# eladb3/SViT

Hardware: AMD Instinct MI355X
Metric: clips/sec (fwd+bwd) SViT 16x224^2 bf16 (higher is better)
Workload: dtype bf16; 1 GPU; SViT 16x224^2, 8 clips/GPU, 4 object tokens/frame, fwd+CE+bwd+clip+AdamW; global_batch=8, parallelism=dp1, ranks_seen=1, forced_dp=False, launch=hip-graph replay, input=fp32 clips, resident in the replayed step's input buffers, hip_library=svit_amd/lib/libsvit_hip.so

## Files before the change

include/svit_hip.h:

```cpp
#ifndef SVIT_HIP_H
#define SVIT_HIP_H
#include <stdint.h>
#ifdef __cplusplus
extern "C" {
#endif

#define SVIT_HEAD_DIM 96

int svit_version(void);
const char* svit_arch(void);

enum {
  SVIT_EPI_BF16 = 0,
  SVIT_EPI_GELU = 1,
  SVIT_EPI_RESID = 2,
  SVIT_EPI_F32 = 3,
  SVIT_EPI_DGELU = 4,
  SVIT_EPI_RELQ = 5
};
typedef struct {
  const void* A; int32_t lda;
  const void* W; int32_t ldw;
  const float* bias;
  void* out; int32_t ldo;
  void* out2; int32_t ldo2;
  const void* aux; int32_t ldaux;
  const float* row_scale; int32_t rows_per_sample;
  int32_t M, N, K;
  int32_t epilogue; int32_t accumulate;
  int32_t remap_L, remap_N, remap_off;
  const int32_t* relq_map;
  void* relq_out; int32_t relq_ld;
  int32_t relq_extra, relq_rows;
  float relq_scale;
} svit_gemm_args;
int svit_gemm_nt(const svit_gemm_args* args, void* stream);
int svit_gemm_tn(const void* A, int lda, const void* B, int ldb, float* dW, int lddw,
                 int M, int N, int K, int splits, float* dbias ,
                 void* stream);
#define SVIT_TN_GROUP_MAX 16
typedef struct {
  const void* A; const void* B; float* dW; float* dbias;
  int32_t lda, ldb, lddw, M, N, K;
} svit_tn_problem;
int svit_gemm_tn_grouped(const svit_tn_problem* probs, int count, void* stream);
int svit_gemm_tn_grouped_ex(const svit_tn_problem* probs, int count, int ordered, void* stream);
int svit_gemm_tn_grouped_slab(const svit_tn_problem* probs, int count, float* workspace,
                              int64_t workspace_floats, void* stream);
int64_t svit_gemm_tn_grouped_workspace(const svit_tn_problem* probs, int count);
int svit_gemm_tn_grouped_slab_lead(const svit_tn_problem* probs, int count, int launch_count, float* workspace,
                                   int64_t workspace_floats, void* stream);
// ... 297 lines not shown
int svit_ce_loss_soft(const float* logits, const float* target, const int64_t* labels, const void* mix, float on,
                      float off, int B, int C, float* loss, float* dlogits, void* stream);
int svit_step_draws(uint64_t* state, const float* keep, int n_blocks, int per_block, float* scales,
                    int n_drop, float p_drop, float* drop, void* stream);

int svit_ensemble_update(const float* preds, const int64_t* labels, const int64_t* clip_ids,
                         int N, int C, int num_clips, int num_videos, int mode, int repeat,
                         float* video_preds, int64_t* video_labels, int64_t* clip_count,
                         int* err, void* stream);
int svit_topk_correct(const float* video_preds, const int64_t* video_labels, int V, int C,
                      const int* ks, int nk, int* counts, int* err, void* stream);
#define SVIT_METER_MAX_SCALARS 16
int svit_meter_push(float* ring, int W, int K, int64_t* state, const float* const* scalars, int n_scalars,
                    const float* logits, const int64_t* labels, int N, int C, int k0, int k1, void* stream);
int svit_debug_set(int key, int val);
int svit_debug_gemm_nt_plan(int M, int N, int K, int epilogue, int32_t* out, int n_out);
int svit_debug_set_tn(int step_us_x100, int atomic_tbs_x100);
int svit_debug_set_tn_tile(int mode);
int svit_debug_gemm_tn_plan(const svit_tn_problem* probs, int count, int form, int arg, int64_t* out, int n_out);
int svit_debug_set_pool(int key, int val);
int svit_debug_pool_bwd_path(void);
int svit_debug_pool_plan(int kind, int B, int heads, int T, int H, int W, int n_obj, int sq, int sk, int sv, int save_mask,
                         int sel, int relq_lpad, int32_t* out, int n_out);
int svit_attn_debug_set(int key, int val);
int svit_debug_reset(void);
#ifdef __cplusplus
}
#endif
#endif
```

svit_amd/build.py:

```python
import concurrent.futures
import os
import re
import subprocess
import sys

HERE = os.path.dirname(os.path.abspath(__file__))
CSRC = os.path.join(HERE, "csrc")
OUT_DIR = os.path.join(HERE, "lib")
LIB = os.path.join(OUT_DIR, "libsvit_hip.so")
SOURCES = ["gemm_nt.hip", "gemm_tn.hip", "norm.hip", "misc.hip", "pool.hip", "attn_fwd.hip", "attn_bwd.hip",
           "loss.hip", "meter.hip", "input.hip", "head.hip", "randaug.hip", "feed.hip", "head_eval.hip", "solver.hip",
           "monitor.hip", "actmon.hip"]
HEADERS = ["common.h", "attn_common.h", "gemm_epilogue.h", os.path.join("..", "..", "include", "svit_hip.h")]
HIPCC = os.environ.get("HIPCC", "/opt/rocm/bin/hipcc")
FLAGS = ["--offload-arch=gfx950", "-O3", "-fPIC", "-std=c++17", "-ffast-math",
         "-fno-finite-math-only", "-fno-slp-vectorize", "-Wno-unused-result"]
SOURCE_FLAGS = {"randaug.hip": {"remove": ["-ffast-math"], "add": ["-ffp-contract=off"]}}
TMP_DIR = os.path.join(OUT_DIR, "tmp")


def flags_for(src):
    change = SOURCE_FLAGS.get(src, {})
    return [f for f in FLAGS if f not in change.get("remove", ())] + list(change.get("add", ()))


# ... 115 lines not shown
```

svit_amd/csrc/common.h:

```cpp
#pragma once
#include <hip/hip_runtime.h>
#include <stdint.h>

typedef uint16_t bf16_t;
typedef __bf16 bf16x8_t __attribute__((ext_vector_type(8)));
typedef __bf16 bf16x4_t __attribute__((ext_vector_type(4)));
typedef short s16x4_t __attribute__((ext_vector_type(4)));
typedef short s16x8_t __attribute__((ext_vector_type(8)));
typedef float f32x16_t __attribute__((ext_vector_type(16)));
typedef float f32x4_t __attribute__((ext_vector_type(4)));

#define SVIT_OK 0
#define SVIT_ERR_SHAPE (-2)
#define SVIT_ERR_ALIGN (-3)
#define SVIT_ERR_ARG (-4)

struct SvitOnce {
  unsigned long long mask;
};
static inline int svit_max_lds_once(SvitOnce& once, const void* fn, size_t bytes) {
  int dev = 0;
  if (hipGetDevice(&dev) != hipSuccess) dev = 0;
  const unsigned long long bit = 1ull << (dev & 63);
  if (__atomic_load_n(&once.mask, __ATOMIC_ACQUIRE) & bit) return 0;
// ... 4 lines not shown
}

enum SvitKnob {
  SVIT_K_NT_STAGES = 0,
  SVIT_K_NT_CFG,
  SVIT_K_NT_BK,
  SVIT_K_TN_STEP_US_X100,
  SVIT_K_TN_ATOMIC_TBS_X100,
  SVIT_K_TN_TILE,
  SVIT_K_POOL_FWD,
  SVIT_K_POOL_BWD,
  SVIT_K_POOL_FWD_LARGE,
  SVIT_K_ATTN_DKV_FORM,
  SVIT_K_ATTN_FWD_SHORT,
  SVIT_K_POOL_FRAME,
  SVIT_K_COUNT
};
int svit_knob(int k);
int svit_knob_set(int k, int v);
void svit_knob_reset();

#define SVIT_LAUNCH_CHECK()                       \
  do {                                            \
    hipError_t e__ = hipGetLastError();           \
    if (e__ != hipSuccess) return (int)e__;       \
  } while (0)

__device__ __forceinline__ float bf16_to_f32(bf16_t v) {
  return __uint_as_float(((uint32_t)v) << 16);
}
// ... 110 lines not shown
```

svit_amd/csrc/gemm_epilogue.h:

```cpp
#pragma once
#include "common.h"
#ifndef SVIT_EPI_AHEAD
#define SVIT_EPI_AHEAD 1
#endif
#include "../../include/svit_hip.h"

template <bool WAVE_PRIVATE>
__device__ __forceinline__ void nt_epi_sync() {
  if constexpr (WAVE_PRIVATE) asm volatile("s_waitcnt lgkmcnt(0)" ::: "memory");
  else __syncthreads();
}

template <int RB, int NB, int EPI, bool WAVE_PRIVATE = false>
__device__ __forceinline__ void nt_epilogue_wide(const svit_gemm_args& p, f32x16_t (&acc)[RB][NB],
                                                 unsigned char* smem, int m0, int n0, int wm, int wn,
                                                 int lane, int wave) {
  constexpr int WN = 32 * NB, EP_LD = WN + 4, GPR = 4 * NB;
  float* stg = (float*)smem + wave * (16 * EP_LD);
  uint4 aux_ring[3][NB];
  auto fetch_aux = [&](int ih, uint4 (&dst)[NB]) {
    const int i = ih >> 1, half = ih & 1;
#pragma unroll
    for (int it = 0; it < NB; ++it) {
      const int idx = lane + 64 * it, rl = idx / GPR, c8 = idx % GPR;
      const int row = m0 + wm * 32 * RB + i * 32 + half * 16 + rl, col = n0 + wn * WN + c8 * 8;
      dst[it] = make_uint4(0, 0, 0, 0);
      if (row < p.M && col < p.N) dst[it] = *(const uint4*)((const bf16_t*)p.aux + (size_t)row * p.ldaux + col);
    }
  };
  float4 bias_r[NB][2];
#pragma unroll
  for (int it = 0; it < NB; ++it) {
    const int col = n0 + wn * WN + ((lane + 64 * it) % GPR) * 8;
    bias_r[it][0] = bias_r[it][1] = make_float4(0.f, 0.f, 0.f, 0.f);
    if (p.bias && col < p.N) {
      bias_r[it][0] = *(const float4*)(p.bias + col);
      bias_r[it][1] = *(const float4*)(p.bias + col + 4);
    }
  }
  constexpr int AHEAD = SVIT_EPI_AHEAD;
  if (EPI == SVIT_EPI_DGELU) {
    fetch_aux(0, aux_ring[0]);
    if (AHEAD > 1 && 2 * RB > 1) fetch_aux(1, aux_ring[1]);
  }
#pragma unroll
  for (int ih = 0; ih < 2 * RB; ++ih) {
    const int i = ih >> 1, half = ih & 1;
#pragma unroll
    for (int j = 0; j < NB; ++j)
#pragma unroll
      for (int rr = 0; rr < 8; ++rr)
        stg[((rr & 3) + 8 * (rr >> 2) + 4 * (lane >> 5)) * EP_LD + j * 32 + (lane & 31)] =
            acc[i][j][half * 8 + rr];
    if (EPI == SVIT_EPI_DGELU && ih + AHEAD < 2 * RB) fetch_aux(ih + AHEAD, aux_ring[(ih + AHEAD) % 3]);
    nt_epi_sync<WAVE_PRIVATE>();
#pragma unroll
    for (int it = 0; it < NB; ++it) {
      const int idx = lane + 64 * it, rl = idx / GPR, c8 = idx % GPR;
      const int row = m0 + wm * 32 * RB + i * 32 + half * 16 + rl, col = n0 + wn * WN + c8 * 8;
      if (row >= p.M || col >= p.N) continue;
      const float4 v0 = *(const float4*)(stg + rl * EP_LD + c8 * 8), v1 = *(const float4*)(stg + rl * EP_LD + c8 * 8 + 4);
      const float4 b0 = bias_r[it][0], b1 = bias_r[it][1];
      float v[8] = {v0.x + b0.x, v0.y + b0.y, v0.z + b0.z, v0.w + b0.w, v1.x + b1.x, v1.y + b1.y, v1.z + b1.z, v1.w + b1.w};
      uint4 o;
      if constexpr (EPI == SVIT_EPI_BF16) {
        o.x = pack_bf16x2(v[0], v[1]); o.y = pack_bf16x2(v[2], v[3]);
        o.z = pack_bf16x2(v[4], v[5]); o.w = pack_bf16x2(v[6], v[7]);
      } else if constexpr (EPI == SVIT_EPI_GELU) {
        float a[8], d[8];
#pragma unroll
        for (int e = 0; e < 8; ++e) gelu_fwd_grad(v[e], &a[e], &d[e]);
        if (p.out2) {
          uint4 o2;
          o2.x = pack_bf16x2(d[0], d[1]); o2.y = pack_bf16x2(d[2], d[3]);
          o2.z = pack_bf16x2(d[4], d[5]); o2.w = pack_bf16x2(d[6], d[7]);
          *(uint4*)((bf16_t*)p.out2 + (size_t)row * p.ldo2 + col) = o2;
        }
        o.x = pack_bf16x2(a[0], a[1]); o.y = pack_bf16x2(a[2], a[3]);
        o.z = pack_bf16x2(a[4], a[5]); o.w = pack_bf16x2(a[6], a[7]);
      } else {
        const uint4 h = aux_ring[ih % 3][it];
        o.x = pack_bf16x2(v[0] * lo_bf16(h.x), v[1] * hi_bf16(h.x));
        o.y = pack_bf16x2(v[2] * lo_bf16(h.y), v[3] * hi_bf16(h.y));
        o.z = pack_bf16x2(v[4] * lo_bf16(h.z), v[5] * hi_bf16(h.z));
        o.w = pack_bf16x2(v[6] * lo_bf16(h.w), v[7] * hi_bf16(h.w));
      }
      *(uint4*)((bf16_t*)p.out + (size_t)row * p.ldo + col) = o;
    }
    if (ih + 1 < 2 * RB) nt_epi_sync<WAVE_PRIVATE>();
  }
}

template <int RB, int NB>
__device__ __forceinline__ void nt_epilogue_relq(const svit_gemm_args& p, f32x16_t (&acc)[RB][NB],
                                                 unsigned char* smem, int m0, int n0, int wm, int wn,
                                                 int lane, int wave) {
  constexpr int WN = 32 * NB, EP_LD = WN + 4;
  constexpr int MAXV = 16;
  float* stg = (float*)smem + wave * (16 * EP_LD);
  const int extra = p.relq_extra, sh = extra == 64 ? 6 : 5;
  const int nv = 16 * extra / 64;
  const int c_lo = n0 + wn * WN;
// ... 177 lines not shown
```

svit_amd/csrc/misc.hip:

```cpp
#include <cstring>
#include <mutex>
#include <unordered_map>
#include "common.h"
#include "../../include/svit_hip.h"

namespace {

__global__ void cast_kernel(const float* __restrict__ src, bf16_t* __restrict__ dst, int64_t n) {
  const int64_t stride = (int64_t)gridDim.x * blockDim.x * 8;
  for (int64_t i = ((int64_t)blockIdx.x * blockDim.x + threadIdx.x) * 8; i < n; i += stride) {
    if (i + 8 <= n) {
      const float4 a = *(const float4*)(src + i), b = *(const float4*)(src + i + 4);
      uint4 o;
      o.x = pack_bf16x2(a.x, a.y); o.y = pack_bf16x2(a.z, a.w);
      o.z = pack_bf16x2(b.x, b.y); o.w = pack_bf16x2(b.z, b.w);
      *(uint4*)(dst + i) = o;
    } else {
      for (int64_t j = i; j < n; ++j) dst[j] = f32_to_bf16(src[j]);
    }
  }
}

__global__ void transpose_cast_kernel(const float* __restrict__ src_base,
                                      bf16_t* __restrict__ dst_base,
// ... 671 lines not shown
  if (!jobs_dev || n_jobs <= 0 || n_jobs > 65535 || max_rows <= 0) return SVIT_ERR_ARG;
  hipLaunchKernelGGL(table_interp_batched_kernel, dim3(max_rows, n_jobs), dim3(128), 0, (hipStream_t)stream, jobs_dev);
  SVIT_LAUNCH_CHECK();
  return SVIT_OK;
}

extern "C" int svit_table_interp(const float* M, int rows, int J, const float* tables, float* out32, void* out16, void* stream) {
  if (!M || !tables || (!out32 && !out16) || rows <= 0 || J <= 0) return SVIT_ERR_ARG;
  hipLaunchKernelGGL(table_interp_kernel, dim3(rows), dim3(128), 0, (hipStream_t)stream, M, J, tables, out32, (bf16_t*)out16);
  SVIT_LAUNCH_CHECK();
  return SVIT_OK;
}

static const int k_knob_default[SVIT_K_COUNT] = {
     0,  -1,  0,  85,  75,  2,
     2,  1,  1,  0,  1,  2};
static int g_knob[SVIT_K_COUNT] = {0, -1, 0, 85, 75, 2, 2, 1, 1, 0, 1, 2};
int svit_knob(int k) { return __atomic_load_n(&g_knob[k], __ATOMIC_RELAXED); }
int svit_knob_set(int k, int v) {
  if (k < 0 || k >= SVIT_K_COUNT) return SVIT_ERR_ARG;
  __atomic_store_n(&g_knob[k], v, __ATOMIC_RELAXED);
  return SVIT_OK;
}
void svit_knob_reset() {
  for (int k = 0; k < SVIT_K_COUNT; ++k) __atomic_store_n(&g_knob[k], k_knob_default[k], __ATOMIC_RELAXED);
}
extern "C" int svit_debug_set(int key, int val) {
  if (key == 0) return (val == 0 || (val >= 2 && val <= 4)) ? svit_knob_set(SVIT_K_NT_STAGES, val) : SVIT_ERR_ARG;
  if (key == 1) return (val >= -1 && val <= 10) ? svit_knob_set(SVIT_K_NT_CFG, val) : SVIT_ERR_ARG;
  if (key == 2) return (val == 0 || val == 32 || val == 64) ? svit_knob_set(SVIT_K_NT_BK, val) : SVIT_ERR_ARG;
  return SVIT_ERR_ARG;
}
extern "C" int svit_debug_set_tn(int step_us_x100, int atomic_tbs_x100) {
  if (step_us_x100 > 0) svit_knob_set(SVIT_K_TN_STEP_US_X100, step_us_x100);
  if (atomic_tbs_x100 > 0) svit_knob_set(SVIT_K_TN_ATOMIC_TBS_X100, atomic_tbs_x100);
  return SVIT_OK;
}
extern "C" int svit_debug_set_tn_tile(int mode) {
  return (mode >= 0 && mode <= 3) ? svit_knob_set(SVIT_K_TN_TILE, mode) : SVIT_ERR_ARG;
}
extern "C" int svit_debug_set_pool(int key, int val) {
  if (key == 0) return (val >= 0 && val <= 3) ? svit_knob_set(SVIT_K_POOL_FWD, val) : SVIT_ERR_ARG;
  if (key == 1) return (val == 0 || val == 1) ? svit_knob_set(SVIT_K_POOL_BWD, val) : SVIT_ERR_ARG;
  if (key == 2) return (val == 0 || val == 1) ? svit_knob_set(SVIT_K_POOL_FWD_LARGE, val) : SVIT_ERR_ARG;
  if (key == 3) return (val >= 0 && val <= 2) ? svit_knob_set(SVIT_K_POOL_FRAME, val) : SVIT_ERR_ARG;
// ... 351 lines not shown
```

svit_amd/engine.py:

```python
import math

import torch

from . import arch, hip, ops
from .augment import AugClips
from .input import FramesView, U8Clips

HD = arch.HEAD_DIM
F32, BF16 = torch.float32, torch.bfloat16
SCALE = HD ** -0.5
LOG2E = 1.4426950408889634
K_SCALE = SCALE * LOG2E


def _align(n, a=8):
    return (n + a - 1) // a * a


class FlatParams:

    @staticmethod
    def layout(shapes, decay_of, rank_of):
        names = list(shapes)
        depth = 1 + max([int(n.split(".")[1]) for n in names if n.startswith("blocks.")] or [0])
# ... 344 lines not shown
        ctx, lse2 = ops.attn_fwd(qa, ka, v, SCALE, bias_cols=J)
        pool_idx = None
        if blk.has_proj:
            skip = ops.gemm_nt(xn2d, f.w(pre + "proj.weight"), f.p(pre + "proj.bias"), hip.EPI_F32)
            skip = skip.view(B, N, Co)
        else:
            skip = x
        if blk.pools_q:
            skip, pool_idx = ops.maxpool_fwd(skip, thw, n_obj)
        dpa, dpm = ds if ds is not None else (None, None)
        x1 = ops.gemm_nt(ctx.view(B * Nq, Co), f.w(pre + "attn.proj.weight"), f.p(pre + "attn.proj.bias"),
                         hip.EPI_RESID, aux=skip.view(B * Nq, Co), row_scale=dpa, rows_per_sample=Nq)
        x1 = x1.view(B, Nq, Co)
        xn2, _, mean2, rstd2 = ops.layernorm_fwd(x1, f.p(pre + "norm2.weight"), f.p(pre + "norm2.bias"),
                                                 save_stats=save)
        act, dact = ops.gemm_nt(xn2.view(B * Nq, Co), f.w(pre + "mlp.fc1.weight"),
                                f.p(pre + "mlp.fc1.bias"), hip.EPI_GELU, save=save)
        x2 = ops.gemm_nt(act, f.w(pre + "mlp.fc2.weight"), f.p(pre + "mlp.fc2.bias"), hip.EPI_RESID,
                         aux=x1.view(B * Nq, Co), row_scale=dpm, rows_per_sample=Nq).view(B, Nq, Co)
        sv = None
        if save:
            sv = dict(x=x, thw=thw, q_thw=q_thw, k_thw=k_thw, mean1=mean1, rstd1=rstd1, xn=xn2d,
                      qkv=qkv, pools=pools, tabs=tabs, idx=idx, mats=mats, ctx=ctx, lse2=lse2,
                      pool_idx=pool_idx, x1=x1, mean2=mean2, rstd2=rstd2, xn2=xn2, act=act,
                      dact=dact, dpa=dpa, dpm=dpm, Nq=Nq)
        return x2, q_thw, sv

    def backward(self, st, dy, on_ready=None, ready_ranks=None):
        def ready(rank):
            if on_ready is not None:
                if ready_ranks is None or rank in ready_ranks:
                    ops.reduce_flush()
                    self._flush_tn()
                    self._join()
# ... 128 lines not shown
        return ops.gemm_nt(dy16, f.wt(wname), None, epilogue, out=out, aux=aux, accumulate=accumulate)

    def _block_bwd(self, blk, sv, dx2, dy, n_obj, below, red_begin=True, red_end=True, red_slot=0):
        f = self.flat
        pre = "blocks.%d." % blk.index
        B, Nq, Co = dx2.shape
        x = sv["x"]
        N, C, h = x.shape[1], x.shape[2], blk.heads
        M, Mq = B * N, B * Nq
        sq, skv = blk.stride_q[1], blk.stride_kv[1]
        thw, q_thw, k_thw = sv["thw"], sv["q_thw"], sv["k_thw"]
        self._red_slot = red_slot
        if red_begin:
            ops.reduce_defer(True)
        dy = dy.view(Mq, Co)
        dh = self._linear_bwd(dy, sv["act"], pre + "mlp.fc2.weight", pre + "mlp.fc2.bias", True,
                              epilogue=hip.EPI_DGELU, aux=sv["dact"])
        dxn2 = self._linear_bwd(dh, sv["xn2"].view(Mq, Co), pre + "mlp.fc1.weight",
                                pre + "mlp.fc1.bias", True, epilogue=hip.EPI_BF16)
        dx1, dy = ops.layernorm_bwd(dxn2, sv["x1"], f.p(pre + "norm2.weight"), sv["mean2"],
                                    sv["rstd2"], f.g(pre + "norm2.weight"), f.g(pre + "norm2.bias"),
                                    dres=dx2, want_bf16=True, row_scale=sv["dpa"], rows_per_sample=Nq,
                                    ws=self._rws("ln2"))
        dy = dy.view(Mq, Co)
        dctx = self._linear_bwd(dy, sv["ctx"].view(Mq, Co), pre + "attn.proj.weight",
                                pre + "attn.proj.bias", True, epilogue=hip.EPI_BF16)
        (qa, preq, mq, rq), (ka, prek, mk, rk), (v, prev, mv, rv) = sv["pools"]
        tabs, mats = sv["tabs"], sv["mats"]
        names = (pre + "attn.rel_pos_h", pre + "attn.rel_pos_w", pre + "attn.rel_pos_t")
        if all(m is None for m in mats):
            rcat_t, lpad, offs = f.rel_cat_t(pre)
        else:
            offs, lpad = rel_sections([t.shape[0] for t in tabs])
            rcat = torch.zeros((lpad, HD), device=self.dev, dtype=F32)
# ... 67 lines not shown
```

svit_amd/hip.py:

```python
import ctypes as C
import os

import torch

_HERE = os.path.dirname(os.path.abspath(__file__))
LIB_PATH = os.environ.get("SVIT_HIP_LIB") or os.path.join(_HERE, "lib", "libsvit_hip.so")
_lib = None

vp, i32, i64, f32 = C.c_void_p, C.c_int32, C.c_int64, C.c_float

EPI_BF16, EPI_GELU, EPI_RESID, EPI_F32, EPI_DGELU, EPI_RELQ = 0, 1, 2, 3, 4, 5


class TnProblem(C.Structure):
    _fields_ = [("A", vp), ("B", vp), ("dW", vp), ("dbias", vp), ("lda", i32), ("ldb", i32),
                ("lddw", i32), ("M", i32), ("N", i32), ("K", i32)]


class GemmArgs(C.Structure):
    _fields_ = [("A", vp), ("lda", i32), ("W", vp), ("ldw", i32), ("bias", vp), ("out", vp),
                ("ldo", i32), ("out2", vp), ("ldo2", i32), ("aux", vp), ("ldaux", i32),
                ("row_scale", vp), ("rows_per_sample", i32), ("M", i32), ("N", i32), ("K", i32),
                ("epilogue", i32), ("accumulate", i32), ("remap_L", i32), ("remap_N", i32),
                ("remap_off", i32), ("relq_map", vp), ("relq_out", vp), ("relq_ld", i32),
                ("relq_extra", i32), ("relq_rows", i32), ("relq_scale", f32)]


class PoolArgs(C.Structure):
    _fields_ = [("qkv", vp), ("which", i32), ("conv_w", vp), ("gamma", vp), ("beta", vp),
                ("out", vp), ("ld_out", i32), ("pre", vp), ("mean", vp), ("rstd", vp),
                ("B", i32), ("heads", i32), ("T", i32), ("H", i32), ("W", i32), ("n_obj", i32),
                ("stride_hw", i32), ("mode", i32), ("eps", f32), ("out_scale", f32),
                ("relq_R", vp), ("relq_map", vp), ("relq_lpad", i32), ("relq_scale", f32)]


class PoolLnBwdArgs(C.Structure):
    _fields_ = [("d_main", vp), ("main_is_f32", i32), ("ld_main", i32), ("d_res", vp),
                ("d_extra", vp), ("pre", vp), ("mean", vp), ("rstd", vp), ("gamma", vp),
                ("dpre", vp), ("dgamma", vp), ("dbeta", vp), ("B", i32), ("heads", i32),
                ("Nout", i32), ("workspace", vp), ("workspace_floats", i64), ("main_parts", i32),
                ("main_part_stride", i64), ("extra_is_bf16", i32)]

# ... 83 lines not shown

class StepHost(C.Structure):
    _fields_ = [("lr", f32 * 2), ("weight_decay", f32 * 2), ("max_norm", f32), ("clip_value", f32),
                ("grad_scale", f32), ("reserved", f32)]


class StepDev(C.Structure):
    _fields_ = [("applied", i64), ("skipped", i64), ("consecutive", i32), ("apply", i32), ("coef", f32),
                ("bc1", f32), ("bc2_sqrt", f32), ("sumsq", f32), ("grad_norm", f32), ("reserved", f32)]


_SIGS = {
    "svit_version": (i32, []),
    "svit_arch": (C.c_char_p, []),
    "svit_gemm_nt": (i32, [C.POINTER(GemmArgs), vp]),
    "svit_gemm_tn": (i32, [vp, i32, vp, i32, vp, i32, i32, i32, i32, i32, vp, vp]),
    "svit_gemm_tn_grouped": (i32, [C.POINTER(TnProblem), i32, vp]),
    "svit_gemm_tn_grouped_ex": (i32, [C.POINTER(TnProblem), i32, i32, vp]),
    "svit_gemm_tn_grouped_slab": (i32, [C.POINTER(TnProblem), i32, vp, i64, vp]),
    "svit_gemm_tn_grouped_workspace": (i64, [C.POINTER(TnProblem), i32]),
    "svit_gemm_tn_grouped_slab_lead": (i32, [C.POINTER(TnProblem), i32, i32, vp, i64, vp]),
    "svit_colsum_bf16": (i32, [vp, i32, vp, i32, i32, vp]),
    "svit_cast_f32_bf16": (i32, [vp, vp, i64, vp]),
    "svit_table_interp": (i32, [vp, i32, i32, vp, vp, vp, vp]),
    "svit_table_interp_batched": (i32, [vp, i32, i32, vp]),
    "svit_transpose_cast_batched": (i32, [vp, vp, vp, i32, i32, vp]),
    "svit_transpose_bf16_batched": (i32, [vp, vp, vp, i32, i32, vp]),
    "svit_scale_cast": (i32, [vp, vp, vp, i32, i64, i32, i32, i32, i32, vp]),
    "svit_pad_cast_rows": (i32, [vp, vp, i32, i32, i32, vp]),
    "svit_reduce_defer": (i32, [i32, vp]),
# ... 65 lines not shown
    "svit_ce_loss": (i32, [vp, vp, i32, i32, vp, vp, vp]),
    "svit_ce_loss_soft": (i32, [vp, vp, vp, vp, f32, f32, i32, i32, vp, vp, vp]),
    "svit_step_draws": (i32, [vp, vp, i32, i32, vp, i32, C.c_float, vp, vp]),
    "svit_ensemble_update": (i32, [vp, vp, vp, i32, i32, i32, i32, i32, i32, vp, vp, vp, vp, vp]),
    "svit_topk_correct": (i32, [vp, vp, i32, i32, vp, i32, vp, vp, vp]),
    "svit_meter_push": (i32, [vp, i32, i32, vp, vp, i32, vp, vp, i32, i32, i32, i32, vp]),
    "svit_debug_set": (i32, [i32, i32]),
    "svit_debug_set_tn": (i32, [i32, i32]),
    "svit_debug_set_tn_tile": (i32, [i32]),
    "svit_debug_set_pool": (i32, [i32, i32]),
    "svit_attn_debug_set": (i32, [i32, i32]),
    "svit_debug_reset": (i32, []),
    "svit_debug_pool_bwd_path": (i32, []),
    "svit_debug_pool_plan": (i32, [i32] * 13 + [C.POINTER(C.c_int32), i32]),
    "svit_debug_gemm_nt_plan": (i32, [i32] * 4 + [C.POINTER(C.c_int32), i32]),
    "svit_debug_gemm_tn_plan": (i32, [C.POINTER(TnProblem), i32, i32, i32, C.POINTER(i64), i32]),
}
EXPORTS = tuple(sorted(_SIGS))


class SvitHipError(RuntimeError):
    pass


def load():
    global _lib
    if _lib is None:
        if not os.path.exists(LIB_PATH):
            raise SvitHipError(
                "libsvit_hip.so not found at %s -- run `python -m svit_amd.build` "
# ... 68 lines not shown
```

svit_amd/ops.py:

```python
import ctypes as C

import torch

from . import hip
from .hip import ptr

BF16 = torch.bfloat16
F32 = torch.float32
HD = 96
_scratch = {}


def scratch(device, floats=8 * 1024 * 1024, tag="main"):
    key = (device.index, floats, tag)
    buf = _scratch.get(key)
    if buf is None:
        buf = torch.empty(floats, device=device, dtype=F32)
        _scratch[key] = buf
    return buf


def _chk_rows(*ts):
    for t in ts:
        if not t.is_cuda or t.dim() != 2 or t.stride(1) != 1:
# ... 59 lines not shown
NT_FAMILIES = ("v2", "ring")
NT_RULES = ("forced", "ring_few_long_tiles", "ring_long_k_narrow", "bk64_narrow_long_k", "one_round_160x256",
            "one_round_192x192", "square_128x128", "big_128x192", "default_128x96")
_NT_PLAN_FIELDS = ("RB", "NB", "WM", "WN", "NL", "stages", "BK", "gx", "gy", "block", "lds")


def gemm_nt_plan(M, N, K, epilogue=hip.EPI_BF16):
    out = (C.c_int32 * 13)()
    n = hip.load().svit_debug_gemm_nt_plan(M, N, K, epilogue, out, 13)
    hip.check(min(n, 0), "svit_debug_gemm_nt_plan")
    plan = dict(zip(_NT_PLAN_FIELDS, out[1:12]))
    plan.update(family=NT_FAMILIES[out[0]], rule=NT_RULES[out[12]])
    return plan


def gemm_tn(a, b, dw, splits=0, dbias=None):
    _chk_rows(a, b)
    _chk_dev(dw)
    M, N = a.shape
    K = dw.shape[-1]
    assert b.shape[0] == M and b.shape[1] >= K and dw.shape[-2] == N and dw.dtype == F32
    hip.call("svit_gemm_tn", ptr(a), a.stride(0), ptr(b), b.stride(0), ptr(dw), dw.stride(-2),
             M, N, K, splits, ptr(dbias), meta=("mnk", M, N, K))
    return dw


def _tn_problem_array(problems):
    arr = (hip.TnProblem * len(problems))()
    flop = 0.0
    for t, (a, b, dw, dbias) in zip(arr, problems):
# ... 1009 lines not shown
```

Baseline: 688.5 clips/s.

## Fuse MLP fc1→GELU→fc2 into a chained GEMM kernel for fwd and bwd

Adds a chained GEMM kernel that computes fc1, applies the GELU (or dGELU) epilogue into an LDS-resident hidden chunk, then multiplies by fc2 in the same workgroup, streaming weight chunks through LDS. The MLP forward and the dgrad path of the MLP backward use this kernel for C=96/192 with H=4C, enabled by default through a new knob. Weight-gradient GEMMs are deferred to the grouped TN list. The aim is to cut the hidden-activation round trip and one launch per MLP. The cost is weight reloads per row tile, since every block rereads the full weights chunk by chunk, and a limit of two workgroups per CU.

Result: no change. 694.1 clips/s (median of 6 runs) (+0.8%).

```diff
diff --git a/include/svit_hip.h b/include/svit_hip.h
--- a/include/svit_hip.h
+++ b/include/svit_hip.h
@@ -35,6 +35,21 @@
   float relq_scale;
 } svit_gemm_args;
 int svit_gemm_nt(const svit_gemm_args* args, void* stream);
+typedef struct {
+  const void* A; int32_t lda;
+  const void* B1; int32_t ldb1;
+  const void* B2; int32_t ldb2;
+  const float* bias1; const float* bias2;
+  void* out_mid; int32_t ld_mid;
+  void* out_mid2; int32_t ld_mid2;
+  const void* aux_mid; int32_t ld_auxmid;
+  void* out; int32_t ldo;
+  const void* aux; int32_t ldaux;
+  const float* row_scale; int32_t rows_per_sample;
+  int32_t M, C, H;
+  int32_t mid, fin;
+} svit_chain_args;
+int svit_gemm_nt_chain(const svit_chain_args* args, void* stream);
 int svit_gemm_tn(const void* A, int lda, const void* B, int ldb, float* dW, int lddw,
                  int M, int N, int K, int splits, float* dbias ,
                  void* stream);
@@ -362,6 +377,7 @@
 int svit_meter_push(float* ring, int W, int K, int64_t* state, const float* const* scalars, int n_scalars,
                     const float* logits, const int64_t* labels, int N, int C, int k0, int k1, void* stream);
 int svit_debug_set(int key, int val);
+int svit_debug_gemm_chain_plan(int M, int C, int H, int mid, int32_t* out, int n_out);
 int svit_debug_gemm_nt_plan(int M, int N, int K, int epilogue, int32_t* out, int n_out);
 int svit_debug_set_tn(int step_us_x100, int atomic_tbs_x100);
 int svit_debug_set_tn_tile(int mode);
diff --git a/svit_amd/build.py b/svit_amd/build.py
--- a/svit_amd/build.py
+++ b/svit_amd/build.py
@@ -8,7 +8,7 @@
 CSRC = os.path.join(HERE, "csrc")
 OUT_DIR = os.path.join(HERE, "lib")
 LIB = os.path.join(OUT_DIR, "libsvit_hip.so")
-SOURCES = ["gemm_nt.hip", "gemm_tn.hip", "norm.hip", "misc.hip", "pool.hip", "attn_fwd.hip", "attn_bwd.hip",
+SOURCES = ["gemm_nt.hip", "gemm_chain.hip", "gemm_tn.hip", "norm.hip", "misc.hip", "pool.hip", "attn_fwd.hip", "attn_bwd.hip",
            "loss.hip", "meter.hip", "input.hip", "head.hip", "randaug.hip", "feed.hip", "head_eval.hip", "solver.hip",
            "monitor.hip", "actmon.hip"]
 HEADERS = ["common.h", "attn_common.h", "gemm_epilogue.h", os.path.join("..", "..", "include", "svit_hip.h")]
diff --git a/svit_amd/csrc/common.h b/svit_amd/csrc/common.h
--- a/svit_amd/csrc/common.h
+++ b/svit_amd/csrc/common.h
@@ -42,6 +42,7 @@
   SVIT_K_ATTN_DKV_FORM,
   SVIT_K_ATTN_FWD_SHORT,
   SVIT_K_POOL_FRAME,
+  SVIT_K_MLP_CHAIN,
   SVIT_K_COUNT
 };
 int svit_knob(int k);
diff --git a/svit_amd/csrc/gemm_chain.hip b/svit_amd/csrc/gemm_chain.hip
--- /dev/null
+++ b/svit_amd/csrc/gemm_chain.hip
@@ -0,0 +1,194 @@
+#include "gemm_epilogue.h"
+
+namespace {
+
+typedef unsigned u32x4_t __attribute__((ext_vector_type(4)));
+
+struct ChainPlan { int bm, hc, lds, wg_per_cu, block; };
+
+template <int C, int HC, int WM, int WN>
+struct ChainGeom {
+  static constexpr int X_LD = HC * 2 + 16;
+  static constexpr int BM = 32 * WM, NT = 64 * WM * WN;
+  static constexpr int NBH = HC / 32 / WN;
+  static constexpr int NBC = C / 32 / WN;
+  static constexpr int W1_LD = C * 2 + 16;
+  static constexpr int W1_BYTES = HC * W1_LD, W2_BYTES = C * X_LD, X_BYTES = BM * X_LD;
+  static constexpr int STG_MID = WM * WN * 16 * (32 * NBH + 4) * 4, STG_FIN = WM * WN * 16 * (32 * NBC + 4) * 4;
+  static constexpr int OFF_W2 = W1_BYTES, OFF_X = OFF_W2 + W2_BYTES, OFF_STG = OFF_X + X_BYTES;
+  static constexpr int LDS = OFF_STG + STG_MID > STG_FIN ? OFF_STG + STG_MID : STG_FIN;
+  static constexpr int PER1 = HC * (C / 8) / NT, PER2 = C * (HC / 8) / NT;
+  static_assert(HC * (C / 8) % NT == 0 && C * (HC / 8) % NT == 0, "whole rounds of 16-B pieces");
+  static_assert(LDS <= 80 * 1024, "two workgroups per CU");
+};
+
+__device__ __forceinline__ void lds_barrier() { asm volatile("s_waitcnt lgkmcnt(0)\n\ts_barrier" ::: "memory"); }
+
+template <int C, int HC, int WM, int WN, int MID, int FIN>
+__global__ __launch_bounds__(64 * WM * WN, 2) void gemm_chain_kernel(svit_chain_args p) {
+  using G = ChainGeom<C, HC, WM, WN>;
+  constexpr int X_LD = G::X_LD;
+  constexpr int NBH = G::NBH, NBC = G::NBC, KS1 = C / 16, KS2 = HC / 16;
+  extern __shared__ __attribute__((aligned(16))) unsigned char smem[];
+  unsigned char* const w1s = smem;
+  unsigned char* const w2s = smem + G::OFF_W2;
+  unsigned char* const xs = smem + G::OFF_X;
+  unsigned char* const stg = smem + G::OFF_STG;
+
+  const int tid = threadIdx.x, lane = tid & 63, wave = tid >> 6;
+  const int wm = wave / WN, wn = wave % WN;
+  const int m0 = blockIdx.x * G::BM;
+  const int r31 = lane & 31, hi = lane >> 5;
+
+  svit_gemm_args p1 = {}, p2 = {};
+  p1.bias = p.bias1, p1.out = p.out_mid, p1.ldo = p.ld_mid, p1.out2 = p.out_mid2, p1.ldo2 = p.ld_mid2;
+  p1.aux = p.aux_mid, p1.ldaux = p.ld_auxmid, p1.M = p.M, p1.N = p.H, p1.K = C;
+  p2.bias = p.bias2, p2.out = p.out, p2.ldo = p.ldo, p2.aux = p.aux, p2.ldaux = p.ldaux;
+  p2.row_scale = p.row_scale, p2.rows_per_sample = p.rows_per_sample, p2.M = p.M, p2.N = C, p2.K = p.H;
+
+  u32x4_t r1[G::PER1], r2[G::PER2];
+  auto fetch_w = [&](int h0) {
+#pragma unroll
+    for (int i = 0; i < G::PER1; ++i) {
+      const int q = tid + i * G::NT, row = q / (C / 8), ch = q % (C / 8);
+      r1[i] = *(const u32x4_t*)((const bf16_t*)p.B1 + (size_t)(h0 + row) * p.ldb1 + ch * 8);
+    }
+#pragma unroll
+    for (int i = 0; i < G::PER2; ++i) {
+      const int q = tid + i * G::NT, row = q / (HC / 8), ch = q % (HC / 8);
+      r2[i] = *(const u32x4_t*)((const bf16_t*)p.B2 + (size_t)row * p.ldb2 + h0 + ch * 8);
+    }
+  };
+  auto put_w1 = [&]() {
+#pragma unroll
+    for (int i = 0; i < G::PER1; ++i) {
+      const int q = tid + i * G::NT, row = q / (C / 8), ch = q % (C / 8);
+      *(u32x4_t*)(w1s + row * G::W1_LD + ch * 16) = r1[i];
+    }
+  };
+  auto put_w2 = [&]() {
+#pragma unroll
+    for (int i = 0; i < G::PER2; ++i) {
+      const int q = tid + i * G::NT, row = q / (HC / 8), ch = q % (HC / 8);
+      *(u32x4_t*)(w2s + row * X_LD + ch * 16) = r2[i];
+    }
+  };
+
+  fetch_w(0);
+  bf16x8_t af[KS1];
+  {
+    const bf16_t* arow = (const bf16_t*)p.A + (size_t)min(m0 + wm * 32 + r31, p.M - 1) * p.lda + 8 * hi;
+#pragma unroll
+    for (int ks = 0; ks < KS1; ++ks) af[ks] = *(const bf16x8_t*)(arow + 16 * ks);
+  }
+  put_w1();
+  put_w2();
+
+  f32x16_t acc2[1][NBC];
+#pragma unroll
+  for (int j = 0; j < NBC; ++j)
+#pragma unroll
+    for (int r = 0; r < 16; ++r) acc2[0][j][r] = 0.f;
+
+  const unsigned char* w1f = w1s + (wn * 32 * NBH + r31) * G::W1_LD + 16 * hi;
+  const unsigned char* w2f = w2s + (wn * 32 * NBC + r31) * X_LD + 16 * hi;
+  const unsigned char* xf = xs + (wm * 32 + r31) * X_LD + 16 * hi;
+
+  uint4 aux_r[2][NBH];
+  auto fetch_aux = [&](int h0) {
+    if constexpr (MID == SVIT_EPI_DGELU) {
+      nt_epi_wide_fetch_aux<1, NBH>(p1, m0, h0, wm, wn, lane, 0, aux_r[0]);
+      nt_epi_wide_fetch_aux<1, NBH>(p1, m0, h0, wm, wn, lane, 1, aux_r[1]);
+    }
+  };
+  fetch_aux(0);
+
+  const int nchunk = p.H / HC;
+  for (int c = 0; c < nchunk; ++c) {
+    const int h0 = c * HC;
+    lds_barrier();
+    if (c + 1 < nchunk) fetch_w(h0 + HC);
+
+    f32x16_t acc1[1][NBH];
+#pragma unroll
+    for (int j = 0; j < NBH; ++j)
+#pragma unroll
+      for (int r = 0; r < 16; ++r) acc1[0][j][r] = 0.f;
+#pragma unroll
+    for (int ks = 0; ks < KS1; ++ks)
+#pragma unroll
+      for (int j = 0; j < NBH; ++j)
+        acc1[0][j] = mfma32(af[ks], *(const bf16x8_t*)(w1f + j * 32 * G::W1_LD + ks * 32), acc1[0][j]);
+
+    nt_epilogue_wide<1, NBH, MID, true>(p1, acc1, stg, m0, h0, wm, wn, lane, wave, xs, X_LD,
+                                        MID == SVIT_EPI_DGELU ? aux_r : nullptr);
+    if (c + 1 < nchunk) fetch_aux(h0 + HC);
+    lds_barrier();
+    if (c + 1 < nchunk) put_w1();
+
+#pragma unroll
+    for (int ks = 0; ks < KS2; ++ks) {
+      const bf16x8_t a = *(const bf16x8_t*)(xf + ks * 32);
+#pragma unroll
+      for (int j = 0; j < NBC; ++j)
+        acc2[0][j] = mfma32(a, *(const bf16x8_t*)(w2f + j * 32 * X_LD + ks * 32), acc2[0][j]);
+    }
+    if (c + 1 < nchunk) {
+      lds_barrier();
+      put_w2();
+    }
+  }
+  lds_barrier();
+  nt_epilogue<1, NBC, FIN, true>(p2, acc2, smem, m0, 0, wm, wn, lane, wave);
+}
+
+typedef void (*ChainKernel)(svit_chain_args);
+struct ChainForm { ChainPlan plan; ChainKernel kernel; SvitOnce once; };
+template <int C, int HC, int WM, int WN, int MID, int FIN>
+constexpr ChainForm chain_form() {
+  using G = ChainGeom<C, HC, WM, WN>;
+  return {{G::BM, HC, G::LDS, (160 * 1024 / G::LDS) < 2 ? 160 * 1024 / G::LDS : 2, G::NT}, gemm_chain_kernel<C, HC, WM, WN, MID, FIN>, {}};
+}
+ChainForm chain_forms[2][2] = {
+    {chain_form<96, 64, 4, 1, SVIT_EPI_GELU, SVIT_EPI_RESID>(), chain_form<96, 64, 4, 1, SVIT_EPI_DGELU, SVIT_EPI_BF16>()},
+    {chain_form<192, 64, 2, 2, SVIT_EPI_GELU, SVIT_EPI_RESID>(), chain_form<192, 32, 4, 1, SVIT_EPI_DGELU, SVIT_EPI_BF16>()}};
+
+ChainForm* chain_choose(int M, int C, int H, int mid) {
+  if (M < 1 || H != 4 * C || (C != 96 && C != 192) || (mid != SVIT_EPI_GELU && mid != SVIT_EPI_DGELU)) return nullptr;
+  return &chain_forms[C == 192][mid == SVIT_EPI_DGELU];
+}
+}
+
+extern "C" int svit_gemm_nt_chain(const svit_chain_args* args, void* stream) {
+  if (!args || !args->A || !args->B1 || !args->B2 || !args->out) return SVIT_ERR_ARG;
+  const svit_chain_args& a = *args;
+  const bool fwd = a.mid == SVIT_EPI_GELU && a.fin == SVIT_EPI_RESID, bwd = a.mid == SVIT_EPI_DGELU && a.fin == SVIT_EPI_BF16;
+  if (!fwd && !bwd) return SVIT_ERR_ARG;
+  if (fwd && (!a.aux || (a.row_scale && a.rows_per_sample <= 0) || (a.out_mid2 && !a.out_mid))) return SVIT_ERR_ARG;
+  if (bwd && (!a.aux_mid || a.bias1 || a.out_mid2)) return SVIT_ERR_ARG;
+  ChainForm* f = chain_choose(a.M, a.C, a.H, a.mid);
+  if (!f) return SVIT_ERR_SHAPE;
+  auto bad_ld = [](int ld, int w) { return ld < w || ld % 8 != 0; };
+  if (bad_ld(a.lda, a.C) || bad_ld(a.ldb1, a.C) || bad_ld(a.ldb2, a.H) || bad_ld(a.ldo, a.C)) return SVIT_ERR_SHAPE;
+  if (a.out_mid && bad_ld(a.ld_mid, a.H)) return SVIT_ERR_SHAPE;
+  if (a.out_mid2 && bad_ld(a.ld_mid2, a.H)) return SVIT_ERR_SHAPE;
+  if (a.aux_mid && bad_ld(a.ld_auxmid, a.H)) return SVIT_ERR_SHAPE;
+  if (fwd && bad_ld(a.ldaux, a.C)) return SVIT_ERR_SHAPE;
+  if (((uintptr_t)a.A | (uintptr_t)a.B1 | (uintptr_t)a.B2 | (uintptr_t)a.out | (uintptr_t)a.out_mid | (uintptr_t)a.out_mid2 |
+       (uintptr_t)a.aux_mid | (uintptr_t)a.aux | (uintptr_t)a.bias1 | (uintptr_t)a.bias2) & 15)
+    return SVIT_ERR_ALIGN;
+  if (int rc = svit_max_lds_once(f->once, (const void*)f->kernel, f->plan.lds)) return rc;
+  const unsigned grid = (unsigned)((a.M + f->plan.bm - 1) / f->plan.bm);
+  hipLaunchKernelGGL(f->kernel, dim3(grid), dim3(f->plan.block), f->plan.lds, (hipStream_t)stream, a);
+  SVIT_LAUNCH_CHECK();
+  return SVIT_OK;
+}
+
+extern "C" int svit_debug_gemm_chain_plan(int M, int C, int H, int mid, int32_t* out, int n_out) {
+  if (!out || n_out < 7) return SVIT_ERR_ARG;
+  const ChainForm* f = chain_choose(M, C, H, mid);
+  if (!f) return SVIT_ERR_SHAPE;
+  out[0] = f->plan.bm, out[1] = f->plan.hc, out[2] = f->plan.lds, out[3] = f->plan.wg_per_cu;
+  out[4] = (M + f->plan.bm - 1) / f->plan.bm, out[5] = f->plan.block, out[6] = svit_knob(SVIT_K_MLP_CHAIN) ? 1 : 0;
+  return 7;
+}
diff --git a/svit_amd/csrc/gemm_epilogue.h b/svit_amd/csrc/gemm_epilogue.h
--- a/svit_amd/csrc/gemm_epilogue.h
+++ b/svit_amd/csrc/gemm_epilogue.h
@@ -11,23 +11,29 @@
   else __syncthreads();
 }
 
+template <int RB, int NB>
+__device__ __forceinline__ void nt_epi_wide_fetch_aux(const svit_gemm_args& p, int m0, int n0, int wm, int wn, int lane,
+                                                      int ih, uint4 (&dst)[NB]) {
+  constexpr int WN = 32 * NB, GPR = 4 * NB;
+  const int i = ih >> 1, half = ih & 1;
+#pragma unroll
+  for (int it = 0; it < NB; ++it) {
+    const int idx = lane + 64 * it, rl = idx / GPR, c8 = idx % GPR;
+    const int row = m0 + wm * 32 * RB + i * 32 + half * 16 + rl, col = n0 + wn * WN + c8 * 8;
+    dst[it] = make_uint4(0, 0, 0, 0);
+    if (row < p.M && col < p.N) dst[it] = *(const uint4*)((const bf16_t*)p.aux + (size_t)row * p.ldaux + col);
+  }
+}
+
 template <int RB, int NB, int EPI, bool WAVE_PRIVATE = false>
 __device__ __forceinline__ void nt_epilogue_wide(const svit_gemm_args& p, f32x16_t (&acc)[RB][NB],
                                                  unsigned char* smem, int m0, int n0, int wm, int wn,
-                                                 int lane, int wave) {
+                                                 int lane, int wave, unsigned char* mid = nullptr, int mid_ld = 0,
+                                                 const uint4 (*pre_aux)[NB] = nullptr) {
   constexpr int WN = 32 * NB, EP_LD = WN + 4, GPR = 4 * NB;
   float* stg = (float*)smem + wave * (16 * EP_LD);
   uint4 aux_ring[3][NB];
-  auto fetch_aux = [&](int ih, uint4 (&dst)[NB]) {
-    const int i = ih >> 1, half = ih & 1;
-#pragma unroll
-    for (int it = 0; it < NB; ++it) {
-      const int idx = lane + 64 * it, rl = idx / GPR, c8 = idx % GPR;
-      const int row = m0 + wm * 32 * RB + i * 32 + half * 16 + rl, col = n0 + wn * WN + c8 * 8;
-      dst[it] = make_uint4(0, 0, 0, 0);
-      if (row < p.M && col < p.N) dst[it] = *(const uint4*)((const bf16_t*)p.aux + (size_t)row * p.ldaux + col);
-    }
-  };
+  auto fetch_aux = [&](int ih, uint4 (&dst)[NB]) { nt_epi_wide_fetch_aux<RB, NB>(p, m0, n0, wm, wn, lane, ih, dst); };
   float4 bias_r[NB][2];
 #pragma unroll
   for (int it = 0; it < NB; ++it) {
@@ -39,7 +45,7 @@
     }
   }
   constexpr int AHEAD = SVIT_EPI_AHEAD;
-  if (EPI == SVIT_EPI_DGELU) {
+  if (EPI == SVIT_EPI_DGELU && !pre_aux) {
     fetch_aux(0, aux_ring[0]);
     if (AHEAD > 1 && 2 * RB > 1) fetch_aux(1, aux_ring[1]);
   }
@@ -52,7 +58,7 @@
       for (int rr = 0; rr < 8; ++rr)
         stg[((rr & 3) + 8 * (rr >> 2) + 4 * (lane >> 5)) * EP_LD + j * 32 + (lane & 31)] =
             acc[i][j][half * 8 + rr];
-    if (EPI == SVIT_EPI_DGELU && ih + AHEAD < 2 * RB) fetch_aux(ih + AHEAD, aux_ring[(ih + AHEAD) % 3]);
+    if (EPI == SVIT_EPI_DGELU && !pre_aux && ih + AHEAD < 2 * RB) fetch_aux(ih + AHEAD, aux_ring[(ih + AHEAD) % 3]);
     nt_epi_sync<WAVE_PRIVATE>();
 #pragma unroll
     for (int it = 0; it < NB; ++it) {
@@ -79,13 +85,14 @@
         o.x = pack_bf16x2(a[0], a[1]); o.y = pack_bf16x2(a[2], a[3]);
         o.z = pack_bf16x2(a[4], a[5]); o.w = pack_bf16x2(a[6], a[7]);
       } else {
-        const uint4 h = aux_ring[ih % 3][it];
+        const uint4 h = pre_aux ? pre_aux[ih][it] : aux_ring[ih % 3][it];
         o.x = pack_bf16x2(v[0] * lo_bf16(h.x), v[1] * hi_bf16(h.x));
         o.y = pack_bf16x2(v[2] * lo_bf16(h.y), v[3] * hi_bf16(h.y));
         o.z = pack_bf16x2(v[4] * lo_bf16(h.z), v[5] * hi_bf16(h.z));
         o.w = pack_bf16x2(v[6] * lo_bf16(h.w), v[7] * hi_bf16(h.w));
       }
-      *(uint4*)((bf16_t*)p.out + (size_t)row * p.ldo + col) = o;
+      if (mid) *(uint4*)(mid + (row - m0) * mid_ld + (col - n0) * 2) = o;
+      if (!mid || p.out) *(uint4*)((bf16_t*)p.out + (size_t)row * p.ldo + col) = o;
     }
     if (ih + 1 < 2 * RB) nt_epi_sync<WAVE_PRIVATE>();
   }
diff --git a/svit_amd/csrc/misc.hip b/svit_amd/csrc/misc.hip
--- a/svit_amd/csrc/misc.hip
+++ b/svit_amd/csrc/misc.hip
@@ -709,8 +709,9 @@
 
 static const int k_knob_default[SVIT_K_COUNT] = {
      0,  -1,  0,  85,  75,  2,
-     2,  1,  1,  0,  1,  2};
-static int g_knob[SVIT_K_COUNT] = {0, -1, 0, 85, 75, 2, 2, 1, 1, 0, 1, 2};
+     2,  1,  1,  0,  1,  2,
+     1};
+static int g_knob[SVIT_K_COUNT] = {0, -1, 0, 85, 75, 2, 2, 1, 1, 0, 1, 2, 1};
 int svit_knob(int k) { return __atomic_load_n(&g_knob[k], __ATOMIC_RELAXED); }
 int svit_knob_set(int k, int v) {
   if (k < 0 || k >= SVIT_K_COUNT) return SVIT_ERR_ARG;
@@ -724,6 +725,7 @@
   if (key == 0) return (val == 0 || (val >= 2 && val <= 4)) ? svit_knob_set(SVIT_K_NT_STAGES, val) : SVIT_ERR_ARG;
   if (key == 1) return (val >= -1 && val <= 10) ? svit_knob_set(SVIT_K_NT_CFG, val) : SVIT_ERR_ARG;
   if (key == 2) return (val == 0 || val == 32 || val == 64) ? svit_knob_set(SVIT_K_NT_BK, val) : SVIT_ERR_ARG;
+  if (key == 3) return (val == 0 || val == 1) ? svit_knob_set(SVIT_K_MLP_CHAIN, val) : SVIT_ERR_ARG;
   return SVIT_ERR_ARG;
 }
 extern "C" int svit_debug_set_tn(int step_us_x100, int atomic_tbs_x100) {
diff --git a/svit_amd/engine.py b/svit_amd/engine.py
--- a/svit_amd/engine.py
+++ b/svit_amd/engine.py
@@ -382,10 +382,17 @@
         x1 = x1.view(B, Nq, Co)
         xn2, _, mean2, rstd2 = ops.layernorm_fwd(x1, f.p(pre + "norm2.weight"), f.p(pre + "norm2.bias"),
                                                  save_stats=save)
-        act, dact = ops.gemm_nt(xn2.view(B * Nq, Co), f.w(pre + "mlp.fc1.weight"),
-                                f.p(pre + "mlp.fc1.bias"), hip.EPI_GELU, save=save)
-        x2 = ops.gemm_nt(act, f.w(pre + "mlp.fc2.weight"), f.p(pre + "mlp.fc2.bias"), hip.EPI_RESID,
-                         aux=x1.view(B * Nq, Co), row_scale=dpm, rows_per_sample=Nq).view(B, Nq, Co)
+        hid = f.w(pre + "mlp.fc1.weight").shape[0]
+        if ops.gemm_nt_chain_ok(B * Nq, Co, hid):
+            x2, act, dact = ops.gemm_nt_chain(xn2.view(B * Nq, Co), f.w(pre + "mlp.fc1.weight"), f.w(pre + "mlp.fc2.weight"),
+                                              hip.EPI_GELU, f.p(pre + "mlp.fc1.bias"), f.p(pre + "mlp.fc2.bias"),
+                                              aux=x1.view(B * Nq, Co), row_scale=dpm, rows_per_sample=Nq, save=save)
+            x2 = x2.view(B, Nq, Co)
+        else:
+            act, dact = ops.gemm_nt(xn2.view(B * Nq, Co), f.w(pre + "mlp.fc1.weight"),
+                                    f.p(pre + "mlp.fc1.bias"), hip.EPI_GELU, save=save)
+            x2 = ops.gemm_nt(act, f.w(pre + "mlp.fc2.weight"), f.p(pre + "mlp.fc2.bias"), hip.EPI_RESID,
+                             aux=x1.view(B * Nq, Co), row_scale=dpm, rows_per_sample=Nq).view(B, Nq, Co)
         sv = None
         if save:
             sv = dict(x=x, thw=thw, q_thw=q_thw, k_thw=k_thw, mean1=mean1, rstd1=rstd1, xn=xn2d,
@@ -544,10 +551,16 @@
         if red_begin:
             ops.reduce_defer(True)
         dy = dy.view(Mq, Co)
-        dh = self._linear_bwd(dy, sv["act"], pre + "mlp.fc2.weight", pre + "mlp.fc2.bias", True,
-                              epilogue=hip.EPI_DGELU, aux=sv["dact"])
-        dxn2 = self._linear_bwd(dh, sv["xn2"].view(Mq, Co), pre + "mlp.fc1.weight",
-                                pre + "mlp.fc1.bias", True, epilogue=hip.EPI_BF16)
+        if ops.gemm_nt_chain_ok(Mq, Co, sv["act"].shape[-1], hip.EPI_DGELU):
+            dxn2, dh = ops.gemm_nt_chain(dy, f.wt(pre + "mlp.fc2.weight"), f.wt(pre + "mlp.fc1.weight"), hip.EPI_DGELU,
+                                         aux_mid=sv["dact"])
+            self._tn.append((dy, sv["act"], f.g(pre + "mlp.fc2.weight"), f.g(pre + "mlp.fc2.bias")))
+            self._tn.append((dh, sv["xn2"].view(Mq, Co), f.g(pre + "mlp.fc1.weight"), f.g(pre + "mlp.fc1.bias")))
+        else:
+            dh = self._linear_bwd(dy, sv["act"], pre + "mlp.fc2.weight", pre + "mlp.fc2.bias", True,
+                                  epilogue=hip.EPI_DGELU, aux=sv["dact"])
+            dxn2 = self._linear_bwd(dh, sv["xn2"].view(Mq, Co), pre + "mlp.fc1.weight",
+                                    pre + "mlp.fc1.bias", True, epilogue=hip.EPI_BF16)
         dx1, dy = ops.layernorm_bwd(dxn2, sv["x1"], f.p(pre + "norm2.weight"), sv["mean2"],
                                     sv["rstd2"], f.g(pre + "norm2.weight"), f.g(pre + "norm2.bias"),
                                     dres=dx2, want_bf16=True, row_scale=sv["dpa"], rows_per_sample=Nq,
diff --git a/svit_amd/hip.py b/svit_amd/hip.py
--- a/svit_amd/hip.py
+++ b/svit_amd/hip.py
@@ -26,6 +26,14 @@
                 ("relq_extra", i32), ("relq_rows", i32), ("relq_scale", f32)]
 
 
+class ChainArgs(C.Structure):
+    _fields_ = [("A", vp), ("lda", i32), ("B1", vp), ("ldb1", i32), ("B2", vp), ("ldb2", i32), ("bias1", vp),
+                ("bias2", vp), ("out_mid", vp), ("ld_mid", i32), ("out_mid2", vp), ("ld_mid2", i32),
+                ("aux_mid", vp), ("ld_auxmid", i32), ("out", vp), ("ldo", i32), ("aux", vp), ("ldaux", i32),
+                ("row_scale", vp), ("rows_per_sample", i32), ("M", i32), ("C", i32), ("H", i32), ("mid", i32),
+                ("fin", i32)]
+
+
 class PoolArgs(C.Structure):
     _fields_ = [("qkv", vp), ("which", i32), ("conv_w", vp), ("gamma", vp), ("beta", vp),
                 ("out", vp), ("ld_out", i32), ("pre", vp), ("mean", vp), ("rstd", vp),
@@ -139,6 +147,7 @@
     "svit_version": (i32, []),
     "svit_arch": (C.c_char_p, []),
     "svit_gemm_nt": (i32, [C.POINTER(GemmArgs), vp]),
+    "svit_gemm_nt_chain": (i32, [C.POINTER(ChainArgs), vp]),
     "svit_gemm_tn": (i32, [vp, i32, vp, i32, vp, i32, i32, i32, i32, i32, vp, vp]),
     "svit_gemm_tn_grouped": (i32, [C.POINTER(TnProblem), i32, vp]),
     "svit_gemm_tn_grouped_ex": (i32, [C.POINTER(TnProblem), i32, i32, vp]),
@@ -234,6 +243,7 @@
     "svit_debug_pool_bwd_path": (i32, []),
     "svit_debug_pool_plan": (i32, [i32] * 13 + [C.POINTER(C.c_int32), i32]),
     "svit_debug_gemm_nt_plan": (i32, [i32] * 4 + [C.POINTER(C.c_int32), i32]),
+    "svit_debug_gemm_chain_plan": (i32, [i32] * 4 + [C.POINTER(C.c_int32), i32]),
     "svit_debug_gemm_tn_plan": (i32, [C.POINTER(TnProblem), i32, i32, i32, C.POINTER(i64), i32]),
 }
 EXPORTS = tuple(sorted(_SIGS))
diff --git a/svit_amd/ops.py b/svit_amd/ops.py
--- a/svit_amd/ops.py
+++ b/svit_amd/ops.py
@@ -97,6 +97,55 @@
     return plan
 
 
+_CHAIN_PLAN_FIELDS = ("tile_rows", "chunk", "lds", "wg_per_cu", "grid", "block", "enabled")
+
+
+def gemm_nt_chain_plan(M, C_, H, mid=hip.EPI_GELU):
+    out = (C.c_int32 * 7)()
+    n = hip.load().svit_debug_gemm_chain_plan(M, C_, H, mid, out, 7)
+    if n == -2:
+        return None
+    hip.check(min(n, 0), "svit_debug_gemm_chain_plan")
+    return dict(zip(_CHAIN_PLAN_FIELDS, out))
+
+
+def gemm_nt_chain_ok(M, C_, H, mid=hip.EPI_GELU):
+    plan = gemm_nt_chain_plan(M, C_, H, mid)
+    return plan is not None and bool(plan["enabled"])
+
+
+def gemm_nt_chain(a, w1, w2, mid, bias1=None, bias2=None, aux_mid=None, aux=None, row_scale=None, rows_per_sample=0,
+                  save=True, out_mid=None, out_mid2=None, out=None):
+    _chk_rows(a)
+    _chk_dev(w1, w2, bias1, bias2, aux_mid, aux, row_scale, out_mid, out_mid2, out)
+    M, Cc = a.shape
+    H = w1.shape[0]
+    assert w1.shape[1] == Cc and w2.shape == (Cc, H) and a.dtype == BF16 and w1.dtype == BF16 and w2.dtype == BF16
+    fwd = mid == hip.EPI_GELU
+    if out is None:
+        out = torch.empty((M, Cc), device=a.device, dtype=F32 if fwd else BF16)
+    if out_mid is None and save:
+        out_mid = torch.empty((M, H), device=a.device, dtype=BF16)
+    if fwd and out_mid2 is None and save:
+        out_mid2 = torch.empty((M, H), device=a.device, dtype=BF16)
+    g = hip.ChainArgs()
+    g.A, g.lda, g.B1, g.ldb1, g.B2, g.ldb2 = ptr(a), a.stride(0), ptr(w1), w1.stride(0), ptr(w2), w2.stride(0)
+    g.bias1, g.bias2 = ptr(bias1), ptr(bias2)
+    g.out_mid, g.ld_mid = ptr(out_mid), (out_mid.stride(-2) if out_mid is not None else 0)
+    g.out_mid2, g.ld_mid2 = ptr(out_mid2), (out_mid2.stride(-2) if out_mid2 is not None else 0)
+    g.aux_mid, g.ld_auxmid = ptr(aux_mid), (aux_mid.stride(-2) if aux_mid is not None else 0)
+    g.out, g.ldo = ptr(out), out.stride(-2)
+    g.aux, g.ldaux = ptr(aux), (aux.stride(-2) if aux is not None else 0)
+    g.row_scale, g.rows_per_sample = ptr(row_scale), rows_per_sample
+    g.M, g.C, g.H, g.mid, g.fin = M, Cc, H, mid, (hip.EPI_RESID if fwd else hip.EPI_BF16)
+    nbytes = 2 * M * Cc + 4 * H * Cc + M * Cc * out.element_size()
+    for t in (out_mid, out_mid2, aux_mid, aux):
+        if t is not None:
+            nbytes += M * t.shape[-1] * t.element_size()
+    hip.call("svit_gemm_nt_chain", C.byref(g), meta=("mnk", M, 2 * H, Cc, mid, nbytes))
+    return (out, out_mid, out_mid2) if fwd else (out, out_mid)
+
+
 def gemm_tn(a, b, dw, splits=0, dbias=None):
     _chk_rows(a, b)
     _chk_dev(dw)
```
